# EPFL-VILAB/omnidata

Measured on AMD Instinct MI355X. Metric: images/sec (384x384) DPT-Hybrid surface-normal inference, higher is better.
Workload: dtype bf16; 1 GPU; DPT-Hybrid-384 normal, batch 32/GPU, bf16, 1xMI355X (BASELINE.json configs[1]); batch_per_gpu=32, global_batch=32, parallelism=replicas x1 (no collective in the loop), ranks_seen=1, inflight=1

## Files before the change

### include/dptx.h

```cpp
#ifndef DPTX_H_
#define DPTX_H_

#include <stddef.h>
#include <stdint.h>

#ifdef __cplusplus
extern "C" {
#endif

typedef struct dptx_engine* dptx_handle;

enum {
  DPTX_OK = 0,
  DPTX_E_INVALID = -1,
  DPTX_E_KEY = -2,
  DPTX_E_HIP = -3,
  DPTX_E_NODEVICE = -4,
  DPTX_E_ALLOC = -5
};

enum { DPTX_DTYPE_BF16 = 0, DPTX_DTYPE_FP16 = 1, DPTX_DTYPE_BF16X3 = 2,
       DPTX_DTYPE_FP16X3 = 3, DPTX_DTYPE_MIXED = 4,
       DPTX_DTYPE_FP8 = 5 };
enum { DPTX_GROUP_RESNET = 1,
// ... 225 lines not shown
int dptx_debug_arena_read(dptx_handle h, void* dst_host, size_t offset, size_t bytes);
int dptx_debug_arena_layout(dptx_handle h, char* dst, size_t capacity);
int dptx_debug_arena_checksums(dptx_handle h, void* out_dev, int32_t capacity, void* stream);
int dptx_debug_set_gemm_flags(int32_t flags);
int dptx_op_conv_fp8(const void* X8, const void* Wt8, const float* bias, const void* R, void* Y, void* Y8, int32_t B,
                     int32_t H, int32_t W, int32_t Cin, int32_t Cout, int32_t ksize, int32_t stride, int32_t pad_t,
                     int32_t pad_l, int32_t Ho, int32_t Wo, int32_t act, int32_t q_relu, float out_scale, void* stream);
int dptx_op_conv_groupnorm(int32_t dtype, const void* X, const void* Wt, void* Yraw, const float* gamma, const float* beta,
                           const void* R, void* Y, int32_t B, int32_t H, int32_t W, int32_t Cin, int32_t Cout,
                           int32_t ksize, int32_t stride, int32_t pad_t, int32_t pad_l, int32_t Ho, int32_t Wo,
                           int32_t relu, float eps, void* scratch_f32, void* stream);
int dptx_op_conv_groupnorm_fused(int32_t dtype, const void* X, const void* Wt, const float* gamma, const float* beta,
                                 const void* R, const float* r_gamma, const float* r_beta, const float* r_records, void* Y,
                                 int32_t B, int32_t H, int32_t W, int32_t Cin, int32_t Cout, int32_t relu, float eps,
                                 void* records_f32, void* tables_f32, int32_t passes, void* stream);
int dptx_op_upsample2x(int32_t dtype, const void* X, void* Y, int32_t B, int32_t H, int32_t W,
                       int32_t C, void* stream);
int dptx_op_gemm_ln(int32_t dtype, const void* A, const void* W, const float* bias, void* C, int32_t M, int32_t N, int32_t K,
                    int32_t act, const float* ln_stats, const float* ln_colsum, int32_t ln_nblk, float ln_eps, void* stream);
int dptx_op_gemm_stream(int32_t dtype, const void* A, const void* W, const float* bias, void* C, float* row_stats, int32_t M,
                        int32_t N, int32_t K, void* stream);
int dptx_op_gemm_stream32(int32_t dtype, const void* A, const void* W, const float* bias, float* X, void* C16, float* row_stats,
                          int32_t M, int32_t N, int32_t K, void* stream);
int dptx_op_head_tail(int32_t dtype, const void* H0, const void* W2, const float* b2, const float* w4,
                      const float* b4, float* y, int32_t B, int32_t Hs, int32_t Ws, int32_t C,
                      int32_t relu_out, void* stream);

typedef struct dptx_unet_engine* dptx_unet_handle;
typedef struct dptx_unet_config {
  int32_t out_channels;
// ... 40 lines not shown
```

### omnidata_amd/build.py

```python
from __future__ import annotations

import os
import subprocess
import sys

HERE = os.path.dirname(os.path.abspath(__file__))
CSRC = os.path.join(HERE, "csrc")
LIB = os.path.join(HERE, "libdptx.so")
SOURCES = ["gemm.hip", "gemm_fp16.hip", "gemm_fp16e.hip", "gemm_x3.hip", "gemm_x2.hip", "gemm_fp8.hip", "conv1x1.hip", "attention.hip", "norm.hip", "misc.hip", "stem.hip", "head.hip", "prepost.hip", "prepost_batch.hip", "fullframe.hip", "refocus.hip", "midas_loss.hip", "vnl_loss.hip", "normal_loss.hip", "eval_metrics.hip", "unet.hip", "unet_engine.hip", "engine.hip", "ops.hip"]
HEADERS = ["common.h", "kernels.h", "gemm_impl.h", "select.h", "unet.h", "resample_batch.h", os.path.join("..", "..", "include", "dptx.h")]
_NOPK = ["-Xclang", "-target-feature", "-Xclang", "-packed-fp32-ops"]
SOURCE_FLAGS = {src: list(_NOPK) for src in ("norm.hip", "misc.hip", "gemm.hip", "gemm_fp16.hip", "gemm_fp16e.hip", "gemm_x3.hip",
                                             "gemm_x2.hip", "gemm_fp8.hip", "conv1x1.hip", "refocus.hip",
                                             "midas_loss.hip", "vnl_loss.hip", "normal_loss.hip", "eval_metrics.hip",
                                             "prepost_batch.hip", "fullframe.hip", "unet.hip")}
EXPERIMENT_HEADERS = []


def source_hash(extra_flags=()) -> str:
    import hashlib
    h = hashlib.sha256()
    for name in sorted(SOURCES + HEADERS + EXPERIMENT_HEADERS):
        path = os.path.join(CSRC, name)
        h.update(os.path.basename(name).encode() + b"\0")
        with open(path, "rb") as f:
# ... 80 lines not shown
```

### omnidata_amd/csrc/conv1x1.hip

```cpp
#include "gemm_impl.h"

namespace dptx {

constexpr int C1_STG_PITCH = 144;
constexpr int C1_STG_WAVE = 16 * C1_STG_PITCH;
constexpr int C1_WAVES = 4;

template <int KT, int BN>
constexpr size_t conv1x1_smem_bytes() {
  return (size_t)KT * BN * 128 + (size_t)C1_WAVES * KT * 32 * 128 + (size_t)C1_WAVES * C1_STG_WAVE;
}

template <int DT>
__device__ __forceinline__ void c1_unpack8(const u32x4_t v, float* f) {
#pragma unroll
  for (int i = 0; i < 4; ++i) {
    f[2 * i] = T16<DT>::tof((uint16_t)(v[i] & 0xffffu));
    f[2 * i + 1] = T16<DT>::tof((uint16_t)(v[i] >> 16));
  }
}

template <int DT, int KT, int BN, int FORM>
__global__ __launch_bounds__(64 * C1_WAVES, KT <= 2 ? 2 : 1) void conv1x1_stream_kernel(const GemmParams p) {
#if defined(__HIP_DEVICE_COMPILE__)
// ... 175 lines not shown
            if (p.act == 1) {
#pragma unroll
              for (int e = 0; e < 8; ++e) f[e] = fmaxf(f[e], 0.f);
            }
#pragma unroll
            for (int e = 0; e < 4; ++e) d[e] = T16<DT>::pack2(f[2 * e], f[2 * e + 1]);
          }
          if (FORM == C1_GN || m < p.M) *(u32x4_t*)((uint16_t*)p.C + (long long)(p.c_row_off + m) * p.ldc + (n0 + s * 64 + cn * 8)) = d;
        }
      }
    }
  }
#endif
}

bool conv1x1_stream_eligible(int mode, const GemmParams& p) {
  if (mode != MODE_BF16 && mode != MODE_FP16) return false;
  if (p.ksz != 1 || p.pad_t != 0 || p.pad_l != 0 || (p.stride != 1 && p.stride != 2)) return false;
  if (p.K != p.Cin || (p.K != 64 && p.K != 128 && p.K != 256) || p.N % 64 != 0) return false;
  if (p.a_fp32 || p.c_fp32 || p.epi2 || p.a_relu || p.R1 != nullptr || p.R2 != nullptr || p.bias_per_img) return false;
  if (p.c_rpi != 0x7fffffff || p.C8 != nullptr || p.C16 != nullptr || p.out_scale != 0.f) return false;
  if (p.row_stats != nullptr || p.ln_stats != nullptr || (p.act != 0 && p.act != 1)) return false;
  if (p.ldc % 8 != 0 || p.a_pix_stride % 8 != 0 || p.a_off % 8 != 0 || p.a_img_stride % 8 != 0) return false;
  if (p.a_bytes <= 0 || p.a_bytes >= (1ll << 31) || (long long)p.N * p.ldw * 2 >= (1ll << 31) || p.M >= (1 << 23)) return false;
  return true;
}

bool conv1x1_stream_adopted(const GemmParams& p) {
  if (p.stride != 1) return false;
  if (p.K == 64) return p.N == 256 || p.N == 64;
// ... 1 lines not shown
  if (p.K == 256) return p.N == 64 || p.N == 128 || (p.N == 256 && p.a_rpi >= 48 * 48);
  return false;
}

bool conv1x1_gn_eligible(int mode, const GemmParams& p) {
  if (!conv1x1_stream_eligible(mode, p) || p.stride != 1 || p.bias != nullptr || p.act != 0) return false;
  const int cpg = p.N / 32;
  if (p.a_rpi % 32 != 0 || p.M % p.a_rpi != 0 || p.N > 1024 || (cpg & (cpg - 1)) != 0) return false;
  return p.c_row_off == 0 && p.ldc == p.N;
}

bool conv1x1_gn_adopted(const GemmParams& p) {
  if (p.K == 64) return p.N == 256;
  if (p.K == 128) return p.N == 512;
  return false;
}

template <int DT, int KT, int BN, int FORM>
static hipError_t launch_c1(const GemmParams& p, hipStream_t stream) {
  constexpr size_t smem = conv1x1_smem_bytes<KT, BN>();
  static_assert(smem <= 160 * 1024 && (KT > 2 || 2 * smem <= 160 * 1024), "two blocks per CU at K <= 128");
  const int npan = p.N / BN;
  const int rb_total = (p.M + 31) / 32;
  const int want = (rb_total + C1_WAVES - 1) / C1_WAVES;
  int cap = (KT <= 2 ? 512 : 256) / npan;
  if (cap < 8) cap = 8;
  int groups = want < cap ? want : cap;
  groups = (groups + 7) / 8 * 8;
  auto k = conv1x1_stream_kernel<DT, KT, BN, FORM>;
  set_smem_attr(k, smem);
// ... 6 lines not shown
  if (p.K == 64) {
    if constexpr (FORM != C1_GN)
      if (p.N % 256 == 0) return launch_c1<DT, 1, 256, FORM>(p, stream);
    if (p.N % 128 == 0) return launch_c1<DT, 1, 128, FORM>(p, stream);
    return launch_c1<DT, 1, 64, FORM>(p, stream);
  }
  if (p.K == 128) return p.N % 128 == 0 ? launch_c1<DT, 2, 128, FORM>(p, stream) : launch_c1<DT, 2, 64, FORM>(p, stream);
  return p.N % 128 == 0 ? launch_c1<DT, 4, 128, FORM>(p, stream) : launch_c1<DT, 4, 64, FORM>(p, stream);
}

template <int FORM>
static hipError_t launch_c1_form(int mode, const GemmParams& p, hipStream_t stream) {
  return mode == MODE_BF16 ? launch_c1_dt<DT_BF16, FORM>(p, stream) : launch_c1_dt<DT_FP16, FORM>(p, stream);
}

hipError_t launch_conv1x1_stream(int mode, const GemmParams& p0, hipStream_t stream, int form) {
  if (form == C1_PLAIN) {
    if (!conv1x1_stream_eligible(mode, p0) || p0.gn_tab != nullptr) return hipErrorInvalidValue;
    return launch_c1_form<C1_PLAIN>(mode, p0, stream);
  }
  GemmParams p = p0;
  p.trace = nullptr;
  p.a_rpi_rcp = 1.0f / (float)(p.a_rpi > 0 ? p.a_rpi : 1);
  p.wout_rcp = 1.0f / (float)(p.Wout > 0 ? p.Wout : 1);
  GemmParams q = p;
  q.R1 = nullptr; q.act = 0; q.gn_tab = nullptr; q.gn_tab_rgn = 0; q.r1_fp32 = 0;
  if (p.M <= 0 || p.ldw < p.K || p.ldw % 8 != 0 || !conv1x1_gn_eligible(mode, q) || p.r1_fp32) return hipErrorInvalidValue;
  p.gn_hw = p.a_rpi; p.gn_blocks = p.a_rpi / 32; p.gn_cpg = p.N / 32;
  if (form == C1_STATS) {
    if (p.gn_part == nullptr || p.R1 != nullptr || p.act != 0 || p.gn_tab != nullptr) return hipErrorInvalidValue;
    return launch_c1_form<C1_STATS>(mode, p, stream);
  }
  if (form != C1_GN || p.gn_tab == nullptr || p.gn_part != nullptr || p.C == nullptr || p.C == p.R1) return hipErrorInvalidValue;
  return launch_c1_form<C1_GN>(mode, p, stream);
}

}
```

### omnidata_amd/csrc/engine.hip

```cpp
#include <hip/hip_runtime.h>

#include <algorithm>
#include <cmath>
#include <cstdio>
#include <chrono>
#include <cstring>
#include <map>
#include <memory>
#include <string>
#include <unordered_map>
#include <vector>

#include "../../include/dptx.h"
#include "kernels.h"

using namespace dptx;

namespace {

constexpr int IMG = 384;
constexpr int S_TOK = 577;
constexpr int FEAT = 256;
const int STAGE_DEPTH[3] = {3, 4, 9};
const int STAGE_OUT[3] = {256, 512, 1024};
// ... 784 lines not shown
    q.gn_part = part;
    exec_macs += macs; cat_macs[0] += macs;
    chk(launch_conv1x1_stream(dt, q, st, C1_STATS), (wkey + ".stats").c_str(), 0);
    const bool r_gn = !rkey.empty();
    chk(launch_gn_finalize(part, e->f(nkey + ".weight"), e->f(nkey + ".bias"), r_gn ? rpart : nullptr,
                           r_gn ? e->f(rkey + ".weight") : nullptr, r_gn ? e->f(rkey + ".bias") : nullptr, tab, B, H * W, Cout,
                           H * W / 32, 1e-5f, st),
        (nkey + ".finalize").c_str(), 2);
    q = p;
    q.R1 = R; q.act = relu; q.gn_tab = tab; q.gn_tab_rgn = r_gn;
    exec_macs += macs; cat_macs[0] += macs;
    chk(launch_conv1x1_stream(dt, q, st, C1_GN), wkey.c_str(), 0);
    return true;
  }

  void rcu(const std::string& p, const void* x, int H, int W, void* tmp, void* out, const GemmOpt& o) {
    const int mid_lo = e->mixed() ? (int)e->layer_reads_lo(p + "conv2.weight", cur_group) : -1;
    conv(x, H, W, FEAT, p + "conv1.weight", 3, 1, 1, 1, H, W, FEAT, tmp,
         GemmOpt().bias(e->f(p + "conv1.bias")).act(1).a_relu(1).q(e->fp8_use(p + "conv2.weight") ? 1 : 0).out_lo(mid_lo));
    conv(tmp, H, W, FEAT, p + "conv2.weight", 3, 1, 1, 1, H, W, FEAT, out,
         GemmOpt().bias(e->f(p + "conv2.bias")).R1(x).R2(o.R2_).q(o.q_).out_lo(e->mixed() ? o.out_lo_ : -1));
  }

  int forward(const void* x, void* y, void* y2);
};

int Run::forward(const void* x, void* y, void* y2) {
  dptx_engine* E = e;
  E->taps.clear();
  E->event_cat.clear();
// ... 43 lines not shown
      const int stride = (b == 0) ? STAGE_STRIDE[s] : 1;
      const int Ho = H / stride, Wo = Wd / stride;
      void* out = (b == STAGE_DEPTH[s] - 1) ? (void*)A(E->S[s]) : (void*)((b & 1) ? A(E->PB) : A(E->PA));
      const bool f_in = gn_fusable(H * Wd), f_out = gn_fusable(Ho * Wo);
      if (b == 0) {
        conv(cur, H, Wd, cin, p + "downsample.conv.weight", 1, stride, 0, 0, Ho, Wo, cout, A(E->DS), GemmOpt().gn_part(f_out ? part3 : nullptr));
        if (!f_out) gn_stats(A(E->DS), part3, Ho * Wo, cout);
      }
      conv(cur, H, Wd, cin, p + "conv1.weight", 1, 1, 0, 0, H, Wd, mid, A(E->T1), GemmOpt().gn_part(f_in ? part0 : nullptr));
      if (!f_in) gn_stats(A(E->T1), part0, H * Wd, mid);
      gn_apply(A(E->T1), p + "norm1", part0, H * Wd, mid, 1);
      const int pad = (stride == 1) ? 1 : 0;
      conv(A(E->T1), H, Wd, mid, p + "conv2.weight", 3, stride, pad, pad, Ho, Wo, mid, A(E->T2), GemmOpt().gn_part(f_out ? part1 : nullptr));
      if (!f_out) gn_stats(A(E->T2), part1, Ho * Wo, mid);
      gn_apply(A(E->T2), p + "norm2", part1, Ho * Wo, mid, 1);
      const bool folded = b == 0 ? conv_gn_folded(A(E->T2), Ho, Wo, mid, p + "conv3.weight", cout, out, p + "norm3", part2, 1, A(E->DS),
                                                  p + "downsample.norm", part3)
                                 : conv_gn_folded(A(E->T2), Ho, Wo, mid, p + "conv3.weight", cout, out, p + "norm3", part2, 1, cur);
      if (!folded) {
        conv(A(E->T2), Ho, Wo, mid, p + "conv3.weight", 1, 1, 0, 0, Ho, Wo, cout, out, GemmOpt().gn_part(f_out ? part2 : nullptr));
        if (!f_out) gn_stats(out, part2, Ho * Wo, cout);
        if (b == 0)
          gn_apply(out, p + "norm3", part2, Ho * Wo, cout, 1, A(E->DS), p + "downsample.norm", part3);
        else
          gn_apply(out, p + "norm3", part2, Ho * Wo, cout, 1, cur);
      }
      cur = out;
      H = Ho;
      Wd = Wo;
      cin = cout;
    }
    const char* names[3] = {"s0", "s1", "s2"};
    tap(names[s], cur, H, Wd, cout);
// ... 921 lines not shown
```

### omnidata_amd/csrc/gemm_impl.h

```cpp
#pragma once
#include <cstdlib>
#include <type_traits>

#include "common.h"
#include "kernels.h"

namespace dptx {

constexpr int BK = 64;

__device__ __forceinline__ int row_div(int m, int d, float rcp, bool big, int& rem) {
  if (big) {
    const int q = m / d;
    rem = m - q * d;
    return q;
  }
  int q = (int)((float)m * rcp);
  int r = m - q * d;
  if (r < 0) { --q; r += d; }
  if (r >= d) { ++q; r -= d; }
  rem = r;
  return q;
}

// ... 106 lines not shown
          if (XT == 3) acc[i][j] = T16<DT>::mfma32(al[s_][i], bf[s_][j], acc[i][j]);
          acc[i][j] = T16<DT>::mfma32(af[s_][i], bl[s_][j], acc[i][j]);
          acc[i][j] = T16<DT>::mfma32(af[s_][i], bf[s_][j], acc[i][j]);
        }
      }
    };
    read(0, 0);
#pragma unroll
    for (int ks = 0; ks < BK / 16; ++ks) {
      if (ks + 1 < BK / 16) read((ks + 1) & 1, ks + 1);
      __builtin_amdgcn_sched_barrier(0);
      mma(ks & 1);
      __builtin_amdgcn_sched_barrier(0);
    }
  }
}

template <int TM, int TN>
__device__ __forceinline__ void gn_records(const GemmParams& p, int m0, int n0, int wm, int wn, int lr, int lh,
                                           f32x16_t (&acc)[TM][TN]) {
  const int cpg = p.gn_cpg;
  const int cpg_sh = __builtin_ctz(cpg);
  int gn_hw = p.gn_hw;
  asm volatile("" : "+s"(gn_hw));
#pragma unroll
  for (int i = 0; i < TM; ++i) {
    const int mb = m0 + (wm * TM + i) * 32;
    const int img = mb / gn_hw;
    const int blk = (mb - img * gn_hw) >> 5;
#pragma unroll
    for (int j = 0; j < TN; ++j) {
      float sm = 0.f, sq = 0.f;
#pragma unroll
      for (int r = 0; r < 16; ++r) { const float v = acc[i][j][r]; sm += v; sq = fmaf(v, v, sq); }
      sm += __shfl_xor(sm, 32, 64);
      sq += __shfl_xor(sq, 32, 64);
      for (int o = 1; o < cpg; o <<= 1) { sm += __shfl_xor(sm, o, 64); sq += __shfl_xor(sq, o, 64); }
      if (lh == 0 && (lr & (cpg - 1)) == 0 && mb < p.M) {
        const int g = (n0 + (wn * TN + j) * 32 + lr) >> cpg_sh;
        float2* dst = (float2*)p.gn_part + ((long long)img * p.gn_blocks + blk) * 32 + g;
        *dst = make_float2(sm, sq);
      }
    }
  }
}

template <int DT, int BM, int BN, int TM, int TN, int PL = 1, int NT = 256, int SLABS = 1, bool WP = false>
__device__ __forceinline__ void epilogue(const GemmParams& p, char* smem, int m0, int n0, int wm, int wn, int lr, int lh,
                                         int tid, f32x16_t (&acc)[TM][TN], int row_pitch = 0, bool dma_in_flight = false,
                                         int trace_row = -1, const char* lds_ln = nullptr) {
  static_assert(SLABS == 1 || SLABS == TM, "one slab, or one per MFMA row tile");
  static_assert(!WP || (SLABS == TM && TN == 2), "wave-private staging: one 32 x 64 block per wave and slab");
  constexpr int CT_PITCH = WP ? 72 : BN + 4;
  constexpr int CT_ROWS = WP ? 32 : BM / SLABS;
  constexpr int NCH = WP ? 8 : BN / 8;
  constexpr int RPP = WP ? 8 : NT / NCH;
// ... 1292 lines not shown
```

### omnidata_amd/csrc/kernels.h

```cpp
#pragma once
#include <hip/hip_runtime.h>
#include <stdint.h>

#include "common.h"

namespace dptx {

void ensure_dyn_smem(const void* kernel, size_t bytes);

struct GemmParams {
  const void* A;
  const void* W;
  void* C;
  const float* bias;
  const void* R1;
  const void* R2;
  int M, N, K;
  int ldw;
  int a_rpi, Wout, Hin, Win, Cin, a_pix_stride;
  long long a_img_stride, a_off;
  long long a_bytes;
  int ksz, stride, pad_t, pad_l;
  int c_rpi, c_img_rows, c_row_off, ldc;
  int r2_bcast;
// ... 26 lines not shown
  int debug_flags;
  float a_rpi_rcp, wout_rcp;
  const float* gn_tab;
  int gn_tab_rgn;
};

void gemm_params_dense(GemmParams& p, int M, int N, int K);
void gemm_params_conv(GemmParams& p, int B, int Hin, int Win, int Cin, int Cout, int ksz, int stride, int pad_t, int pad_l,
                      int Hout, int Wout, int a_elem_bytes);
hipError_t launch_gemm(int dtype, const GemmParams& p, hipStream_t stream);
void gemm_set_trace(long long* dev_buf);
void gemm_set_debug_flags(int flags);
int gemm_debug_flags();
bool conv1x1_stream_eligible(int mode, const GemmParams& p);
bool conv1x1_stream_adopted(const GemmParams& p);
enum { C1_PLAIN = 0, C1_STATS = 1, C1_GN = 2 };
bool conv1x1_gn_eligible(int mode, const GemmParams& p);
bool conv1x1_gn_adopted(const GemmParams& p);
hipError_t launch_conv1x1_stream(int mode, const GemmParams& p, hipStream_t stream, int form = C1_PLAIN);
void gemm_set_cu_share(float share);

hipError_t launch_attention(int mode, const void* qkv, void* out, int B, int S, int heads, Planes pl, hipStream_t stream);

hipError_t launch_layernorm(int mode, const float* x, const float* gamma, const float* beta, void* y,
                            int M, int C, float eps, Planes pl, hipStream_t stream);

struct GnParams {
  const void* X; void* Y;
  const float* gamma; const float* beta;
  float* partial;
  const void* R;
  const float* r_gamma; const float* r_beta; const float* r_partial;
  int B, HW, C, relu;
  float eps;
// ... 43 lines not shown
```

### omnidata_amd/csrc/norm.hip

```cpp
#include "common.h"
#include "kernels.h"

namespace dptx {

template <int DT, int PL, int VPL>
__global__ __launch_bounds__(256) void layernorm_kernel(const float* __restrict__ x, const float* __restrict__ gamma,
                                                        const float* __restrict__ beta, uint16_t* __restrict__ y,
                                                        int M, int C, float eps, long long plane) {
  const int lane = threadIdx.x & 63;
  const int row = blockIdx.x * 4 + (threadIdx.x >> 6);
  if (row >= M) return;
  const float* xr = x + (long long)row * C;
  float4 v[VPL];
  float s = 0.f;
#pragma unroll
  for (int j = 0; j < VPL; ++j) {
    v[j] = *(const float4*)(xr + (j * 64 + lane) * 4);
    s += (v[j].x + v[j].y) + (v[j].z + v[j].w);
  }
  const float mean = wave_sum(s) / (float)C;
  float q = 0.f;
#pragma unroll
  for (int j = 0; j < VPL; ++j) {
    const float a = v[j].x - mean, b = v[j].y - mean, c = v[j].z - mean, d = v[j].w - mean;
// ... 98 lines not shown
  if (C % 64 != 0 || C > 1024 || (256 % (C / 8)) != 0) return hipErrorInvalidValue;
  dim3 grid(gn_chunks(HW, C), B);
  DPTX_DISPATCH_MODE(mode, hipLaunchKernelGGL((gn_stats_kernel<DT, PL>), grid, dim3(256), 0, stream, (const uint16_t*)X, partial,
                                              HW, C, gn_pix(C), pl.act));
  return hipGetLastError();
}

__device__ __forceinline__ void gn_affine_to_lds(const float* __restrict__ partial, int nchunks, int b,
                                                 const float* __restrict__ gamma, const float* __restrict__ beta, int C,
                                                 int HW, float eps, float* sa, float* sd, float* smr) {
  __shared__ double sred[8][GN_G][2];
  const int tid = threadIdx.x;
  const int cpg = C >> 5;
  {
    const int g = tid & (GN_G - 1), slice = tid >> 5;
    double ss = 0.0, qq = 0.0;
    const float2* pp = (const float2*)partial + (long long)b * nchunks * GN_G + g;
    for (int c = slice; c < nchunks; c += 8) {
      const float2 v = pp[(long long)c * GN_G];
      ss += (double)v.x;
      qq += (double)v.y;
    }
    sred[slice][g][0] = ss;
    sred[slice][g][1] = qq;
  }
  __syncthreads();
  if (tid < GN_G) {
    double ss = 0.0, qq = 0.0;
#pragma unroll
    for (int sl = 0; sl < 8; ++sl) { ss += sred[sl][tid][0]; qq += sred[sl][tid][1]; }
    const double n = (double)HW * (double)cpg;
    const double mean = ss / n;
    double var = qq / n - mean * mean;
    if (var < 0.0) var = 0.0;
    smr[2 * tid] = (float)mean;
    smr[2 * tid + 1] = (float)(1.0 / sqrt(var + (double)eps));
  }
  __syncthreads();
  for (int c = tid; c < C; c += blockDim.x) {
    const int g = c / cpg;
    const float a = __fmul_rn(smr[2 * g + 1], gamma[c]);
    sa[c] = a;
    sd[c] = __builtin_fmaf(-a, smr[2 * g], beta[c]);
  }
  __syncthreads();
}

template <int DT, int PL>
__global__ __launch_bounds__(256) void gn_apply_kernel(const GnParams p, int pix, int nrec, long long plane) {
  __shared__ float sa[1024], sd[1024], ra[1024], rd[1024], smr[64];
  const int b = blockIdx.y;
  gn_affine_to_lds(p.partial, nrec, b, p.gamma, p.beta, p.C, p.HW, p.eps, sa, sd, smr);
  const bool r_gn = (p.R != nullptr) && (p.r_gamma != nullptr);
  if (r_gn) gn_affine_to_lds(p.r_partial, nrec, b, p.r_gamma, p.r_beta, p.C, p.HW, p.eps, ra, rd, smr);
  const int cvec = p.C >> 3;
  const int pbeg = blockIdx.x * pix;
  const int pend = min(pbeg + pix, p.HW);
  const long long img = (long long)b * p.HW * p.C;
// ... 117 lines not shown
```

### omnidata_amd/csrc/ops.hip

```cpp
#include <hip/hip_runtime.h>

#include "../../include/dptx.h"
#include "kernels.h"

using namespace dptx;

extern "C" {

static int rc(hipError_t r) { return r == hipSuccess ? DPTX_OK : DPTX_E_HIP; }

static Planes g_op_planes{0, 0};
int dptx_op_set_planes(int64_t act_plane_elems, int64_t w_plane_elems) {
  g_op_planes.act = act_plane_elems;
  g_op_planes.w = w_plane_elems;
  return DPTX_OK;
}

int dptx_op_gemm(int32_t dtype, const void* A, const void* W, const float* bias, const void* R, void* C, int32_t M, int32_t N,
                 int32_t K, int32_t act, int32_t a_fp32, int32_t c_fp32, int32_t r_fp32, void* stream) {
  GemmParams p;
  gemm_params_dense(p, M, N, K);
  p.A = A; p.W = W; p.C = C; p.bias = bias; p.R1 = R; p.act = act; p.a_fp32 = a_fp32; p.c_fp32 = c_fp32; p.r1_fp32 = r_fp32;
  p.planes = g_op_planes;
  return rc(launch_gemm(dtype, p, (hipStream_t)stream));
// ... 141 lines not shown
    if (launch_conv1x1_stream(dtype, q, st, C1_STATS) != hipSuccess) return DPTX_E_HIP;
  }
  if (passes & 2) {
    if (launch_gn_finalize((const float*)records_f32, gamma, beta, r_records, r_gamma, r_beta, (float*)tables_f32, B, H * W, Cout,
                           H * W / 32, eps, st) != hipSuccess)
      return DPTX_E_HIP;
  }
  if (passes & 4) {
    GemmParams q = p;
    q.R1 = R; q.act = relu ? 1 : 0; q.gn_tab = (const float*)tables_f32; q.gn_tab_rgn = r_gamma != nullptr;
    if (launch_conv1x1_stream(dtype, q, st, C1_GN) != hipSuccess) return DPTX_E_HIP;
  }
  return DPTX_OK;
}

int dptx_op_upsample2x(int32_t dtype, const void* X, void* Y, int32_t B, int32_t H, int32_t W, int32_t C, void* stream) {
  return rc(launch_upsample2x(dtype, X, Y, B, H, W, C, g_op_planes, (hipStream_t)stream));
}

}
```

### omnidata_amd/engine.py

```python
from __future__ import annotations

import ctypes as C
import os
from typing import Dict, Optional, Tuple

import numpy as np
import torch

_HERE = os.path.dirname(os.path.abspath(__file__))
LIB_PATH = os.environ.get("DPTX_LIB") or os.path.join(_HERE, "libdptx.so")

DTYPES = {"bf16": 0, "fp16": 1, "bf16x3": 2, "fp16x3": 3, "mixed": 4, "fp8": 5}
TWO_PLANE_DTYPES = frozenset(("bf16x3", "fp16x3", "mixed", "fp8"))
GROUPS = {"resnet": 1, "embed": 2, "vit": 4, "reassemble": 8, "rn": 16, "fusion": 32, "head": 64, "all": 127}
FLAGS = {"no_ln_fold": 1, "group_policy": 2, "fp32_stream": 4, "no_range_check": 8, "fp8_all": 16, "fp8_vit": 32}


def groups_mask(names) -> int:
    if isinstance(names, int):
        return names
    if isinstance(names, str):
        names = [n for n in names.replace(",", "+").split("+") if n]
    mask = 0
    for n in names:
# ... 95 lines not shown
    ("dptx_op_stem_conv", C.c_int, [_i32, _vp, _vp, _vp, _i32, _i32, _i32, _vp]),
    ("dptx_op_attention", C.c_int, [_i32, _vp, _vp, _i32, _i32, _i32, _vp]),
    ("dptx_op_layernorm", C.c_int, [_i32, _vp, _vp, _vp, _vp, _i32, _i32, C.c_float, _vp]),
    ("dptx_op_groupnorm", C.c_int, [_i32, _vp, _vp, _vp, _vp, _vp, _i32, _i32, _i32, _i32, C.c_float, _vp, _vp]),
    ("dptx_op_gn_relu_maxpool", C.c_int, [_i32, _vp, _vp, _vp, _vp, _i32, _i32, _i32, _i32, C.c_float, _vp, _vp]),
    ("dptx_op_cls_rows", C.c_int, [_i32, _vp, _vp, _vp, _i32, _i32, _i32, _vp, _vp, _vp, C.c_float, _vp]),
    ("dptx_debug_set_trace", C.c_int, [_vp]),
    ("dptx_debug_set_gemm_flags", C.c_int, [C.c_int32]),
    ("dptx_debug_arena_fill", C.c_int, [_vp, _i32]),
    ("dptx_debug_arena_read", C.c_int, [_vp, _vp, _sz, _sz]),
    ("dptx_debug_arena_layout", C.c_int, [_vp, C.c_char_p, _sz]),
    ("dptx_debug_arena_checksums", C.c_int, [_vp, _vp, _i32, _vp]),
    ("dptx_op_conv_fp8", C.c_int, [_vp, _vp, _vp, _vp, _vp, _vp] + [_i32] * 13 + [C.c_float, _vp]),
    ("dptx_op_conv_groupnorm", C.c_int, [_i32, _vp, _vp, _vp, _vp, _vp, _vp, _vp] + [_i32] * 12 + [C.c_float, _vp, _vp]),
    ("dptx_op_conv_groupnorm_fused", C.c_int, [_i32] + [_vp] * 9 + [_i32] * 6 + [C.c_float, _vp, _vp, _i32, _vp]),
    ("dptx_op_upsample2x", C.c_int, [_i32, _vp, _vp, _i32, _i32, _i32, _i32, _vp]),
    ("dptx_op_gemm_ln", C.c_int, [_i32, _vp, _vp, _vp, _vp, _i32, _i32, _i32, _i32, _vp, _vp, _i32, C.c_float, _vp]),
    ("dptx_op_gemm_stream", C.c_int, [_i32, _vp, _vp, _vp, _vp, _vp, _i32, _i32, _i32, _vp]),
    ("dptx_op_gemm_stream32", C.c_int, [_i32, _vp, _vp, _vp, _vp, _vp, _vp, _i32, _i32, _i32, _vp]),
    ("dptx_op_head_tail", C.c_int, [_i32, _vp, _vp, _vp, _vp, _vp, _vp, _i32, _i32, _i32, _i32, _i32, _vp]),
    ("dptx_unet_default_config", None, [_vp]),
    ("dptx_unet_create", C.c_int, [C.POINTER(_vp), _vp]),
    ("dptx_unet_destroy", None, [_vp]),
    ("dptx_unet_last_error", C.c_char_p, [_vp]),
    ("dptx_unet_load_tensor", C.c_int, [_vp, C.c_char_p, _vp, _i64p, _i32]),
    ("dptx_unet_finalize_weights", C.c_int, [_vp]),
    ("dptx_unet_packed_bytes", _sz, [_vp]),
    ("dptx_unet_packed_entry", C.c_int, [_vp, C.c_char_p, _i64p, _i64p]),
    ("dptx_unet_export_packed_host", C.c_int, [_vp, _vp, _sz]),
    ("dptx_unet_device_bytes", _sz, [_vp]),
# ... 368 lines not shown
```

Measured before the change: 2868 images/s.

## Fuse 1x1 conv with whole-image GroupNorm in a single per-image kernel

```diff
diff --git a/include/dptx.h b/include/dptx.h
--- a/include/dptx.h
+++ b/include/dptx.h
@@ -263,6 +263,9 @@
                                  const void* R, const float* r_gamma, const float* r_beta, const float* r_records, void* Y,
                                  int32_t B, int32_t H, int32_t W, int32_t Cin, int32_t Cout, int32_t relu, float eps,
                                  void* records_f32, void* tables_f32, int32_t passes, void* stream);
+int dptx_op_conv_groupnorm_image(int32_t dtype, const void* X, const void* Wt, const float* gamma, const float* beta,
+                                 const void* R, const float* r_gamma, const float* r_beta, const float* r_records, void* Y,
+                                 int32_t B, int32_t H, int32_t W, int32_t Cin, int32_t Cout, int32_t relu, float eps, void* stream);
 int dptx_op_upsample2x(int32_t dtype, const void* X, void* Y, int32_t B, int32_t H, int32_t W,
                        int32_t C, void* stream);
 int dptx_op_gemm_ln(int32_t dtype, const void* A, const void* W, const float* bias, void* C, int32_t M, int32_t N, int32_t K,
diff --git a/omnidata_amd/build.py b/omnidata_amd/build.py
--- a/omnidata_amd/build.py
+++ b/omnidata_amd/build.py
@@ -8,7 +8,7 @@
 CSRC = os.path.join(HERE, "csrc")
 LIB = os.path.join(HERE, "libdptx.so")
 SOURCES = ["gemm.hip", "gemm_fp16.hip", "gemm_fp16e.hip", "gemm_x3.hip", "gemm_x2.hip", "gemm_fp8.hip", "conv1x1.hip", "attention.hip", "norm.hip", "misc.hip", "stem.hip", "head.hip", "prepost.hip", "prepost_batch.hip", "fullframe.hip", "refocus.hip", "midas_loss.hip", "vnl_loss.hip", "normal_loss.hip", "eval_metrics.hip", "unet.hip", "unet_engine.hip", "engine.hip", "ops.hip"]
-HEADERS = ["common.h", "kernels.h", "gemm_impl.h", "select.h", "unet.h", "resample_batch.h", os.path.join("..", "..", "include", "dptx.h")]
+HEADERS = ["common.h", "kernels.h", "gemm_impl.h", "gn_affine.h", "select.h", "unet.h", "resample_batch.h", os.path.join("..", "..", "include", "dptx.h")]
 _NOPK = ["-Xclang", "-target-feature", "-Xclang", "-packed-fp32-ops"]
 SOURCE_FLAGS = {src: list(_NOPK) for src in ("norm.hip", "misc.hip", "gemm.hip", "gemm_fp16.hip", "gemm_fp16e.hip", "gemm_x3.hip",
                                              "gemm_x2.hip", "gemm_fp8.hip", "conv1x1.hip", "refocus.hip",
diff --git a/omnidata_amd/csrc/conv1x1.hip b/omnidata_amd/csrc/conv1x1.hip
--- a/omnidata_amd/csrc/conv1x1.hip
+++ b/omnidata_amd/csrc/conv1x1.hip
@@ -1,4 +1,5 @@
 #include "gemm_impl.h"
+#include "gn_affine.h"
 
 namespace dptx {
 
@@ -213,6 +214,268 @@
 #endif
 }
 
+constexpr int C1_IMG_RB = 5;
+constexpr int C1_IMG_REC = C1_WAVES * C1_IMG_RB;
+constexpr int C1_IMG_MAX_ROWS = C1_IMG_REC * 32;
+
+struct C1ImgArgs {
+  const float *gamma, *beta;
+  const float *r_gamma, *r_beta, *r_part;
+  float eps;
+};
+
+template <int KT>
+constexpr size_t conv1x1_img_smem_bytes() {
+  return (size_t)KT * 64 * 128 + (size_t)C1_WAVES * KT * 32 * 128 + (size_t)C1_WAVES * C1_STG_WAVE;
+}
+
+template <int KT>
+__device__ __forceinline__ void c1_issue_a(const GemmParams& p, const __amdgpu_buffer_rsrc_t rsrcA, char* sa, int lane, int rblk) {
+  const int kc = lane & 7, r0 = lane >> 3;
+#pragma unroll
+  for (int i = 0; i < 4; ++i) {
+    const int row = r0 + 8 * i;
+    const int m = rblk * 32 + row;
+    const bool ok = m < p.M;
+    const int mm = ok ? m : 0;
+    int rem, ox;
+    const int img = row_div(mm, p.a_rpi, p.a_rpi_rcp, false, rem);
+    const int oy = row_div(rem, p.Wout, p.wout_rcp, false, ox);
+    const int iy = oy * p.stride - p.pad_t, ix = ox * p.stride - p.pad_l;
+    const bool valid = ok && ((unsigned)iy < (unsigned)p.Hin) && ((unsigned)ix < (unsigned)p.Win);
+    const long long e = (long long)img * p.a_img_stride + p.a_off + ((long long)iy * p.Win + ix) * p.a_pix_stride +
+                        (kc ^ ((row >> 1) & 7)) * 8;
+    const unsigned base = (unsigned)(e * 2);
+#pragma unroll
+    for (int kt = 0; kt < KT; ++kt) {
+      const unsigned vo = valid ? base + kt * 128 : OOB;
+      __builtin_amdgcn_raw_ptr_buffer_load_lds(rsrcA, (__attribute__((address_space(3))) void*)(sa + kt * 4096 + i * 1024), 16, vo,
+                                               0, 0, 0);
+    }
+  }
+}
+
+template <int DT, int KT>
+__global__ __launch_bounds__(64 * C1_WAVES, 1) void conv1x1_image_kernel(const GemmParams p, const C1ImgArgs g) {
+#if defined(__HIP_DEVICE_COMPILE__)
+  constexpr int BN = 64;
+  constexpr int KS = KT * 4;
+  constexpr int W_BYTES = KT * BN * 128;
+  constexpr int A_WAVE = KT * 32 * 128;
+  constexpr int RB = C1_IMG_RB;
+  extern __shared__ __attribute__((aligned(16))) char smem[];
+  __shared__ float2 s_rec[C1_IMG_REC][32];
+  __shared__ double s_red[2][8][32][2];
+  __shared__ float s_mr[2][64];
+  __shared__ float s_aff[4][BN];
+
+  const int tid = threadIdx.x;
+  const int lane = tid & 63;
+  const int wave = __builtin_amdgcn_readfirstlane(tid >> 6);
+  const int lr = lane & 31, lh = lane >> 5;
+
+  const int npan = p.N / BN;
+  const int x = (int)blockIdx.x & 7, l = (int)blockIdx.x >> 3;
+  const int img = (l / npan) * 8 + x;
+  const int n0 = (l % npan) * BN;
+  const int nrb = p.gn_blocks;
+  if (img * p.gn_hw >= p.M) return;
+  const int rbase = img * nrb;
+
+  const int cpg = p.gn_cpg, cpg_sh = __builtin_ctz(cpg);
+  const int gpp = BN >> cpg_sh;
+  const bool has_r = p.R1 != nullptr;
+  const bool r_gn = has_r && g.r_part != nullptr;
+
+  const int w_bytes = (int)((long long)p.N * p.ldw * 2);
+  const __amdgpu_buffer_rsrc_t rsrcA = __builtin_amdgcn_make_buffer_rsrc(const_cast<void*>(p.A), 0, (int)p.a_bytes, 0x00020000);
+  const __amdgpu_buffer_rsrc_t rsrcW = __builtin_amdgcn_make_buffer_rsrc(const_cast<void*>(p.W), 0, w_bytes, 0x00020000);
+  char* const sw = smem;
+  char* const sa = smem + W_BYTES + wave * A_WAVE;
+  char* const stg = smem + W_BYTES + C1_WAVES * A_WAVE + wave * C1_STG_WAVE;
+
+  if (wave < nrb) c1_issue_a<KT>(p, rsrcA, sa, lane, rbase + wave);
+  {
+    const int kc = lane & 7, r0 = lane >> 3;
+    for (int idx = wave; idx < KT * (BN / 8); idx += C1_WAVES) {
+      const int kt = idx / (BN / 8), rg = idx - kt * (BN / 8);
+      const int row = rg * 8 + r0;
+      const unsigned vo = (unsigned)(((long long)(n0 + row) * p.ldw + kt * 64 + (kc ^ ((row >> 1) & 7)) * 8) * 2);
+      __builtin_amdgcn_raw_ptr_buffer_load_lds(rsrcW, (__attribute__((address_space(3))) void*)(sw + kt * (BN * 128) + rg * 1024), 16,
+                                               vo, 0, 0, 0);
+    }
+  }
+  const int sg = tid & 31, slice = tid >> 5;
+  const int at = tid >> 6, ac = tid & 63;
+  float gam = 0.f, bet = 0.f;
+  if (at == 0 || (at == 1 && r_gn)) {
+    gam = (at ? g.r_gamma : g.gamma)[n0 + ac];
+    bet = (at ? g.r_beta : g.beta)[n0 + ac];
+  }
+  if (r_gn && sg < gpp) {
+    double ss, qq;
+    gn_slice_sums((const float2*)g.r_part + (long long)rbase * 32 + (n0 >> cpg_sh) + sg, 32, nrb, slice, ss, qq);
+    s_red[1][slice][sg][0] = ss;
+    s_red[1][slice][sg][1] = qq;
+  }
+  asm volatile("s_waitcnt vmcnt(0)" ::: "memory");
+  __syncthreads();
+
+  const int swz = (lr >> 1) & 7;
+  const unsigned sel = (lr & 1) ? 0x03020706u : 0x05040100u;
+  const int cn = lane & 7, rr = lane >> 3;
+
+  uint32_t pk[RB][2][8];
+  u32x4_t rq[RB][4];
+  float2 rs[RB * 2];
+#pragma unroll
+  for (int n = 0; n < RB * 2; ++n) rs[n] = make_float2(0.f, 0.f);
+#pragma unroll
+  for (int i = 0; i < RB; ++i) {
+    const int rb = wave + C1_WAVES * i;
+    if (rb < nrb) {
+      const int m0 = (rbase + rb) * 32;
+      u32x4_t af[KS];
+#pragma unroll
+      for (int ks = 0; ks < KS; ++ks)
+        af[ks] = *(const u32x4_t*)(sa + (ks >> 2) * 4096 + lr * 128 + (((2 * (ks & 3) + lh) ^ swz) << 4));
+      asm volatile("s_waitcnt lgkmcnt(0)" ::: "memory");
+      const bool prefetch = rb + C1_WAVES < nrb;
+      if (prefetch) c1_issue_a<KT>(p, rsrcA, sa, lane, rbase + rb + C1_WAVES);
+      asm volatile("" ::: "memory");
+      if (has_r) {
+#pragma unroll
+        for (int q = 0; q < 4; ++q) {
+          const int m = m0 + 16 * (q >> 1) + rr + 8 * (q & 1);
+          rq[i][q] = *(const u32x4_t*)((const uint16_t*)p.R1 + (long long)m * p.ldc + (n0 + cn * 8));
+        }
+      }
+      asm volatile("" ::: "memory");
+
+      f32x16_t acc[2];
+#pragma unroll
+      for (int j = 0; j < 2; ++j)
+#pragma unroll
+        for (int r = 0; r < 16; ++r) acc[j][r] = 0.f;
+      u32x4_t bf[2][4][2];
+      auto read_w = [&](int kt) {
+#pragma unroll
+        for (int q = 0; q < 4; ++q)
+#pragma unroll
+          for (int j = 0; j < 2; ++j)
+            bf[kt & 1][q][j] = *(const u32x4_t*)(sw + kt * (BN * 128) + (j * 32 + lr) * 128 + (((2 * q + lh) ^ swz) << 4));
+      };
+      read_w(0);
+#pragma unroll
+      for (int kt = 0; kt < KT; ++kt) {
+        if (kt + 1 < KT) read_w(kt + 1);
+        __builtin_amdgcn_sched_barrier(0);
+#pragma unroll
+        for (int q = 0; q < 4; ++q)
+#pragma unroll
+          for (int j = 0; j < 2; ++j) acc[j] = T16<DT>::mfma32(af[kt * 4 + q], bf[kt & 1][q][j], acc[j]);
+      }
+      __builtin_amdgcn_sched_barrier(0);
+#pragma unroll
+      for (int j = 0; j < 2; ++j) {
+        rs[2 * i + j] = gn_record_rows(acc[j]);
+#pragma unroll
+        for (int t = 0; t < 8; ++t) pk[i][j][t] = T16<DT>::pack2(acc[j][2 * t], acc[j][2 * t + 1]);
+      }
+      if (prefetch) {
+        if (has_r) asm volatile("s_waitcnt vmcnt(4)" ::: "memory");
+        else asm volatile("s_waitcnt vmcnt(0)" ::: "memory");
+      }
+    }
+  }
+  gn_record_lanes<RB * 2>(rs, cpg);
+#pragma unroll
+  for (int i = 0; i < RB; ++i) {
+    const int rb = wave + C1_WAVES * i;
+#pragma unroll
+    for (int j = 0; j < 2; ++j)
+      if (rb < nrb && lh == 0 && (lr & (cpg - 1)) == 0) s_rec[rb][(j * 32 + lr) >> cpg_sh] = rs[2 * i + j];
+  }
+  __syncthreads();
+
+  if (sg < gpp) {
+    double ss, qq;
+    gn_slice_sums(&s_rec[0][sg], 32, nrb, slice, ss, qq);
+    s_red[0][slice][sg][0] = ss;
+    s_red[0][slice][sg][1] = qq;
+  }
+  __syncthreads();
+  if (tid < 64 && sg < gpp && (slice == 0 || r_gn))
+    gn_mean_rstd(&s_red[slice][0][sg][0], 64, p.gn_hw, cpg, g.eps, s_mr[slice][2 * sg], s_mr[slice][2 * sg + 1]);
+  __syncthreads();
+  if (at == 0 || (at == 1 && r_gn)) {
+    const int gg = ac >> cpg_sh;
+    gn_channel_affine(s_mr[at][2 * gg], s_mr[at][2 * gg + 1], gam, bet, s_aff[2 * at][ac], s_aff[2 * at + 1][ac]);
+  }
+  __syncthreads();
+
+  float ga[8], gd[8], gra[8], grd[8];
+#pragma unroll
+  for (int e = 0; e < 8; ++e) {
+    ga[e] = s_aff[0][cn * 8 + e];
+    gd[e] = s_aff[1][cn * 8 + e];
+    gra[e] = r_gn ? s_aff[2][cn * 8 + e] : 0.f;
+    grd[e] = r_gn ? s_aff[3][cn * 8 + e] : 0.f;
+  }
+#pragma unroll
+  for (int i = 0; i < RB; ++i) {
+    const int rb = wave + C1_WAVES * i;
+    if (rb < nrb) {
+      const int m0 = (rbase + rb) * 32;
+#pragma unroll
+      for (int h = 0; h < 2; ++h) {
+        asm volatile("" ::: "memory");
+        __builtin_amdgcn_wave_barrier();
+#pragma unroll
+        for (int j = 0; j < 2; ++j)
+#pragma unroll
+          for (int t = 0; t < 4; ++t) {
+            const uint32_t own = pk[i][j][4 * h + t];
+            const uint32_t nb = (uint32_t)__builtin_amdgcn_update_dpp(0, (int)own, 0xB1, 0xf, 0xf, false);
+            const uint32_t o = __builtin_amdgcn_perm(nb, own, sel);
+            const int rl = ((2 * t) & 3) + (lr & 1) + 8 * (t >> 1) + 4 * lh;
+            *(uint32_t*)(stg + rl * C1_STG_PITCH + (j * 32 + (lr & ~1)) * 2) = o;
+          }
+        asm volatile("" ::: "memory");
+        __builtin_amdgcn_wave_barrier();
+#pragma unroll
+        for (int pp = 0; pp < 2; ++pp) {
+          const int rl = rr + 8 * pp;
+          u32x4_t d = *(const u32x4_t*)(stg + rl * C1_STG_PITCH + cn * 16);
+          const int m = m0 + 16 * h + rl;
+          float f[8];
+          c1_unpack8<DT>(d, f);
+#pragma unroll
+          for (int e = 0; e < 8; ++e) f[e] = __builtin_fmaf(f[e], ga[e], gd[e]);
+          if (has_r) {
+            float r[8];
+            c1_unpack8<DT>(rq[i][2 * h + pp], r);
+            if (r_gn) {
+#pragma unroll
+              for (int e = 0; e < 8; ++e) r[e] = __builtin_fmaf(r[e], gra[e], grd[e]);
+            }
+#pragma unroll
+            for (int e = 0; e < 8; ++e) f[e] = __fadd_rn(f[e], r[e]);
+          }
+          if (p.act == 1) {
+#pragma unroll
+            for (int e = 0; e < 8; ++e) f[e] = fmaxf(f[e], 0.f);
+          }
+#pragma unroll
+          for (int e = 0; e < 4; ++e) d[e] = T16<DT>::pack2(f[2 * e], f[2 * e + 1]);
+          *(u32x4_t*)((uint16_t*)p.C + (long long)m * p.ldc + (n0 + cn * 8)) = d;
+        }
+      }
+    }
+  }
+#endif
+}
+
 bool conv1x1_stream_eligible(int mode, const GemmParams& p) {
   if (mode != MODE_BF16 && mode != MODE_FP16) return false;
   if (p.ksz != 1 || p.pad_t != 0 || p.pad_l != 0 || (p.stride != 1 && p.stride != 2)) return false;
@@ -244,6 +507,33 @@
   if (p.K == 64) return p.N == 256;
   if (p.K == 128) return p.N == 512;
   return false;
+}
+
+bool conv1x1_gn_image_eligible(int mode, const GemmParams& p) {
+  return conv1x1_gn_eligible(mode, p) && p.a_rpi <= C1_IMG_MAX_ROWS;
+}
+
+bool conv1x1_gn_image_adopted(const GemmParams& p) {
+  return p.K == 256 && p.N == 1024 && p.a_rpi <= C1_IMG_MAX_ROWS;
+}
+
+template <int DT, int KT>
+static hipError_t launch_c1_img(const GemmParams& p, const C1ImgArgs& g, hipStream_t stream) {
+  constexpr size_t smem = conv1x1_img_smem_bytes<KT>();
+  static_assert(smem + 16 * 1024 <= 160 * 1024, "dynamic + static LDS of conv1x1_image_kernel");
+  const int npan = p.N / 64;
+  const int nimg = p.M / p.a_rpi;
+  auto k = conv1x1_image_kernel<DT, KT>;
+  set_smem_attr(k, smem);
+  hipLaunchKernelGGL(k, dim3((nimg + 7) / 8 * 8 * npan), dim3(64 * C1_WAVES), smem, stream, p, g);
+  return hipGetLastError();
+}
+
+template <int DT>
+static hipError_t launch_c1_img_dt(const GemmParams& p, const C1ImgArgs& g, hipStream_t stream) {
+  if (p.K == 64) return launch_c1_img<DT, 1>(p, g, stream);
+  if (p.K == 128) return launch_c1_img<DT, 2>(p, g, stream);
+  return launch_c1_img<DT, 4>(p, g, stream);
 }
 
 template <int DT, int KT, int BN, int FORM>
@@ -280,7 +570,7 @@
   return mode == MODE_BF16 ? launch_c1_dt<DT_BF16, FORM>(p, stream) : launch_c1_dt<DT_FP16, FORM>(p, stream);
 }
 
-hipError_t launch_conv1x1_stream(int mode, const GemmParams& p0, hipStream_t stream, int form) {
+hipError_t launch_conv1x1_stream(int mode, const GemmParams& p0, hipStream_t stream, int form, const GnParams* gn) {
   if (form == C1_PLAIN) {
     if (!conv1x1_stream_eligible(mode, p0) || p0.gn_tab != nullptr) return hipErrorInvalidValue;
     return launch_c1_form<C1_PLAIN>(mode, p0, stream);
@@ -293,6 +583,13 @@
   q.R1 = nullptr; q.act = 0; q.gn_tab = nullptr; q.gn_tab_rgn = 0; q.r1_fp32 = 0;
   if (p.M <= 0 || p.ldw < p.K || p.ldw % 8 != 0 || !conv1x1_gn_eligible(mode, q) || p.r1_fp32) return hipErrorInvalidValue;
   p.gn_hw = p.a_rpi; p.gn_blocks = p.a_rpi / 32; p.gn_cpg = p.N / 32;
+  if (form == C1_IMG) {
+    if (gn == nullptr || gn->gamma == nullptr || gn->beta == nullptr || !conv1x1_gn_image_eligible(mode, q)) return hipErrorInvalidValue;
+    if (p.gn_part != nullptr || p.gn_tab != nullptr || p.C == nullptr || p.C == p.R1) return hipErrorInvalidValue;
+    if (gn->r_partial != nullptr && (p.R1 == nullptr || gn->r_gamma == nullptr || gn->r_beta == nullptr)) return hipErrorInvalidValue;
+    const C1ImgArgs g{gn->gamma, gn->beta, gn->r_gamma, gn->r_beta, gn->r_partial, gn->eps};
+    return mode == MODE_BF16 ? launch_c1_img_dt<DT_BF16>(p, g, stream) : launch_c1_img_dt<DT_FP16>(p, g, stream);
+  }
   if (form == C1_STATS) {
     if (p.gn_part == nullptr || p.R1 != nullptr || p.act != 0 || p.gn_tab != nullptr) return hipErrorInvalidValue;
     return launch_c1_form<C1_STATS>(mode, p, stream);
diff --git a/omnidata_amd/csrc/engine.hip b/omnidata_amd/csrc/engine.hip
--- a/omnidata_amd/csrc/engine.hip
+++ b/omnidata_amd/csrc/engine.hip
@@ -822,6 +822,25 @@
     return true;
   }
 
+  bool conv_gn_image(const void* in, int H, int W, int Cin, const std::string& wkey, int Cout, void* out, const std::string& nkey,
+                     int relu, const void* R, const std::string& rkey = "", const float* rpart = nullptr) {
+    const int flags = gemm_debug_flags();
+    if ((flags & (8 | 32 | 64)) || !gn_fusable(H * W) || out == R || (e->fp8_use(wkey) && !e->calibrating)) return false;
+    GemmParams p;
+    gemm_params_conv(p, B, H, W, Cin, Cout, 1, 1, 0, 0, H, W, 2);
+    p.A = in; p.W = e->w(wkey); p.C = out; p.planes = e->pl;
+    if (!conv1x1_gn_image_eligible(dt, p) || !((flags & 128) || conv1x1_gn_image_adopted(p))) return false;
+    const bool r_gn = !rkey.empty();
+    GnParams g{};
+    g.gamma = e->f(nkey + ".weight"); g.beta = e->f(nkey + ".bias"); g.eps = 1e-5f;
+    if (r_gn) { g.r_gamma = e->f(rkey + ".weight"); g.r_beta = e->f(rkey + ".bias"); g.r_partial = rpart; }
+    p.R1 = R; p.act = relu;
+    const double macs = (double)p.M / B * p.N * p.K;
+    exec_macs += macs; cat_macs[0] += macs;
+    chk(launch_conv1x1_stream(dt, p, st, C1_IMG, &g), wkey.c_str(), 0);
+    return true;
+  }
+
   void rcu(const std::string& p, const void* x, int H, int W, void* tmp, void* out, const GemmOpt& o) {
     const int mid_lo = e->mixed() ? (int)e->layer_reads_lo(p + "conv2.weight", cur_group) : -1;
     conv(x, H, W, FEAT, p + "conv1.weight", 3, 1, 1, 1, H, W, FEAT, tmp,
@@ -895,9 +914,11 @@
       conv(A(E->T1), H, Wd, mid, p + "conv2.weight", 3, stride, pad, pad, Ho, Wo, mid, A(E->T2), GemmOpt().gn_part(f_out ? part1 : nullptr));
       if (!f_out) gn_stats(A(E->T2), part1, Ho * Wo, mid);
       gn_apply(A(E->T2), p + "norm2", part1, Ho * Wo, mid, 1);
-      const bool folded = b == 0 ? conv_gn_folded(A(E->T2), Ho, Wo, mid, p + "conv3.weight", cout, out, p + "norm3", part2, 1, A(E->DS),
-                                                  p + "downsample.norm", part3)
-                                 : conv_gn_folded(A(E->T2), Ho, Wo, mid, p + "conv3.weight", cout, out, p + "norm3", part2, 1, cur);
+      const void* R = b == 0 ? (const void*)A(E->DS) : cur;
+      const std::string rkey = b == 0 ? p + "downsample.norm" : std::string();
+      const float* rpart = b == 0 ? part3 : nullptr;
+      const bool folded = conv_gn_image(A(E->T2), Ho, Wo, mid, p + "conv3.weight", cout, out, p + "norm3", 1, R, rkey, rpart) ||
+                          conv_gn_folded(A(E->T2), Ho, Wo, mid, p + "conv3.weight", cout, out, p + "norm3", part2, 1, R, rkey, rpart);
       if (!folded) {
         conv(A(E->T2), Ho, Wo, mid, p + "conv3.weight", 1, 1, 0, 0, Ho, Wo, cout, out, GemmOpt().gn_part(f_out ? part2 : nullptr));
         if (!f_out) gn_stats(out, part2, Ho * Wo, cout);
diff --git a/omnidata_amd/csrc/gemm_impl.h b/omnidata_amd/csrc/gemm_impl.h
--- a/omnidata_amd/csrc/gemm_impl.h
+++ b/omnidata_amd/csrc/gemm_impl.h
@@ -144,6 +144,30 @@
       __builtin_amdgcn_sched_barrier(0);
     }
   }
+}
+
+__device__ __forceinline__ float2 gn_record_rows(const f32x16_t& a) {
+  float sm = 0.f, sq = 0.f;
+#pragma unroll
+  for (int r = 0; r < 16; ++r) { const float v = a[r]; sm += v; sq = fmaf(v, v, sq); }
+  return make_float2(sm, sq);
+}
+template <int NREC>
+__device__ __forceinline__ void gn_record_lanes(float2 (&s)[NREC], int cpg) {
+#pragma unroll
+  for (int n = 0; n < NREC; ++n) {
+    s[n].x += __shfl_xor(s[n].x, 32, 64);
+    s[n].y += __shfl_xor(s[n].y, 32, 64);
+  }
+  for (int o = 1; o < cpg; o <<= 1) {
+#pragma unroll
+    for (int n = 0; n < NREC; ++n) { s[n].x += __shfl_xor(s[n].x, o, 64); s[n].y += __shfl_xor(s[n].y, o, 64); }
+  }
+}
+__device__ __forceinline__ float2 gn_record_sums(const f32x16_t& a, int cpg) {
+  float2 s[1] = {gn_record_rows(a)};
+  gn_record_lanes<1>(s, cpg);
+  return s[0];
 }
 
 template <int TM, int TN>
@@ -160,16 +184,11 @@
     const int blk = (mb - img * gn_hw) >> 5;
 #pragma unroll
     for (int j = 0; j < TN; ++j) {
-      float sm = 0.f, sq = 0.f;
-#pragma unroll
-      for (int r = 0; r < 16; ++r) { const float v = acc[i][j][r]; sm += v; sq = fmaf(v, v, sq); }
-      sm += __shfl_xor(sm, 32, 64);
-      sq += __shfl_xor(sq, 32, 64);
-      for (int o = 1; o < cpg; o <<= 1) { sm += __shfl_xor(sm, o, 64); sq += __shfl_xor(sq, o, 64); }
+      const float2 rec = gn_record_sums(acc[i][j], cpg);
       if (lh == 0 && (lr & (cpg - 1)) == 0 && mb < p.M) {
         const int g = (n0 + (wn * TN + j) * 32 + lr) >> cpg_sh;
         float2* dst = (float2*)p.gn_part + ((long long)img * p.gn_blocks + blk) * 32 + g;
-        *dst = make_float2(sm, sq);
+        *dst = rec;
       }
     }
   }
diff --git a/omnidata_amd/csrc/gn_affine.h b/omnidata_amd/csrc/gn_affine.h
--- /dev/null
+++ b/omnidata_amd/csrc/gn_affine.h
@@ -0,0 +1,33 @@
+#pragma once
+#include "common.h"
+
+namespace dptx {
+
+__device__ __forceinline__ void gn_slice_sums(const float2* rec, int stride, int nrec, int slice, double& ss, double& qq) {
+  ss = 0.0;
+  qq = 0.0;
+  for (int c = slice; c < nrec; c += 8) {
+    const float2 v = rec[(long long)c * stride];
+    ss += (double)v.x;
+    qq += (double)v.y;
+  }
+}
+
+__device__ __forceinline__ void gn_mean_rstd(const double* sred, int stride, int HW, int cpg, float eps, float& mean, float& rstd) {
+  double ss = 0.0, qq = 0.0;
+#pragma unroll
+  for (int sl = 0; sl < 8; ++sl) { ss += sred[sl * stride]; qq += sred[sl * stride + 1]; }
+  const double n = (double)HW * (double)cpg;
+  const double m = ss / n;
+  double var = qq / n - m * m;
+  if (var < 0.0) var = 0.0;
+  mean = (float)m;
+  rstd = (float)(1.0 / sqrt(var + (double)eps));
+}
+
+__device__ __forceinline__ void gn_channel_affine(float mean, float rstd, float gamma, float beta, float& a, float& d) {
+  a = __fmul_rn(rstd, gamma);
+  d = __builtin_fmaf(-a, mean, beta);
+}
+
+}
diff --git a/omnidata_amd/csrc/kernels.h b/omnidata_amd/csrc/kernels.h
--- a/omnidata_amd/csrc/kernels.h
+++ b/omnidata_amd/csrc/kernels.h
@@ -64,10 +64,13 @@
 int gemm_debug_flags();
 bool conv1x1_stream_eligible(int mode, const GemmParams& p);
 bool conv1x1_stream_adopted(const GemmParams& p);
-enum { C1_PLAIN = 0, C1_STATS = 1, C1_GN = 2 };
+enum { C1_PLAIN = 0, C1_STATS = 1, C1_GN = 2, C1_IMG = 3 };
+struct GnParams;
 bool conv1x1_gn_eligible(int mode, const GemmParams& p);
 bool conv1x1_gn_adopted(const GemmParams& p);
-hipError_t launch_conv1x1_stream(int mode, const GemmParams& p, hipStream_t stream, int form = C1_PLAIN);
+bool conv1x1_gn_image_eligible(int mode, const GemmParams& p);
+bool conv1x1_gn_image_adopted(const GemmParams& p);
+hipError_t launch_conv1x1_stream(int mode, const GemmParams& p, hipStream_t stream, int form = C1_PLAIN, const GnParams* gn = nullptr);
 void gemm_set_cu_share(float share);
 
 hipError_t launch_attention(int mode, const void* qkv, void* out, int B, int S, int heads, Planes pl, hipStream_t stream);
diff --git a/omnidata_amd/csrc/norm.hip b/omnidata_amd/csrc/norm.hip
--- a/omnidata_amd/csrc/norm.hip
+++ b/omnidata_amd/csrc/norm.hip
@@ -1,4 +1,5 @@
 #include "common.h"
+#include "gn_affine.h"
 #include "kernels.h"
 
 namespace dptx {
@@ -136,34 +137,17 @@
   const int cpg = C >> 5;
   {
     const int g = tid & (GN_G - 1), slice = tid >> 5;
-    double ss = 0.0, qq = 0.0;
-    const float2* pp = (const float2*)partial + (long long)b * nchunks * GN_G + g;
-    for (int c = slice; c < nchunks; c += 8) {
-      const float2 v = pp[(long long)c * GN_G];
-      ss += (double)v.x;
-      qq += (double)v.y;
-    }
+    double ss, qq;
+    gn_slice_sums((const float2*)partial + (long long)b * nchunks * GN_G + g, GN_G, nchunks, slice, ss, qq);
     sred[slice][g][0] = ss;
     sred[slice][g][1] = qq;
   }
   __syncthreads();
-  if (tid < GN_G) {
-    double ss = 0.0, qq = 0.0;
-#pragma unroll
-    for (int sl = 0; sl < 8; ++sl) { ss += sred[sl][tid][0]; qq += sred[sl][tid][1]; }
-    const double n = (double)HW * (double)cpg;
-    const double mean = ss / n;
-    double var = qq / n - mean * mean;
-    if (var < 0.0) var = 0.0;
-    smr[2 * tid] = (float)mean;
-    smr[2 * tid + 1] = (float)(1.0 / sqrt(var + (double)eps));
-  }
+  if (tid < GN_G) gn_mean_rstd(&sred[0][tid][0], GN_G * 2, HW, cpg, eps, smr[2 * tid], smr[2 * tid + 1]);
   __syncthreads();
   for (int c = tid; c < C; c += blockDim.x) {
     const int g = c / cpg;
-    const float a = __fmul_rn(smr[2 * g + 1], gamma[c]);
-    sa[c] = a;
-    sd[c] = __builtin_fmaf(-a, smr[2 * g], beta[c]);
+    gn_channel_affine(smr[2 * g], smr[2 * g + 1], gamma[c], beta[c], sa[c], sd[c]);
   }
   __syncthreads();
 }
diff --git a/omnidata_amd/csrc/ops.hip b/omnidata_amd/csrc/ops.hip
--- a/omnidata_amd/csrc/ops.hip
+++ b/omnidata_amd/csrc/ops.hip
@@ -179,6 +179,23 @@
   return DPTX_OK;
 }
 
+int dptx_op_conv_groupnorm_image(int32_t dtype, const void* X, const void* Wt, const float* gamma, const float* beta, const void* R,
+                                 const float* r_gamma, const float* r_beta, const float* r_records, void* Y, int32_t B, int32_t H,
+                                 int32_t W, int32_t Cin, int32_t Cout, int32_t relu, float eps, void* stream) {
+  if (X == nullptr || Wt == nullptr || gamma == nullptr || beta == nullptr || Y == nullptr || Y == R || B <= 0 || H <= 0 || W <= 0)
+    return DPTX_E_INVALID;
+  if ((r_gamma != nullptr) != (r_beta != nullptr) || (r_gamma != nullptr) != (r_records != nullptr)) return DPTX_E_INVALID;
+  if (r_gamma != nullptr && R == nullptr) return DPTX_E_INVALID;
+  GemmParams p;
+  gemm_params_conv(p, B, H, W, Cin, Cout, 1, 1, 0, 0, H, W, 2);
+  p.A = X; p.W = Wt; p.C = Y; p.planes = g_op_planes;
+  if (!conv1x1_gn_image_eligible(dtype, p)) return DPTX_E_INVALID;
+  GnParams g{};
+  g.gamma = gamma; g.beta = beta; g.r_gamma = r_gamma; g.r_beta = r_beta; g.r_partial = r_records; g.eps = eps;
+  p.R1 = R; p.act = relu ? 1 : 0;
+  return rc(launch_conv1x1_stream(dtype, p, (hipStream_t)stream, C1_IMG, &g));
+}
+
 int dptx_op_upsample2x(int32_t dtype, const void* X, void* Y, int32_t B, int32_t H, int32_t W, int32_t C, void* stream) {
   return rc(launch_upsample2x(dtype, X, Y, B, H, W, C, g_op_planes, (hipStream_t)stream));
 }
diff --git a/omnidata_amd/engine.py b/omnidata_amd/engine.py
--- a/omnidata_amd/engine.py
+++ b/omnidata_amd/engine.py
@@ -133,6 +133,7 @@
     ("dptx_op_conv_fp8", C.c_int, [_vp, _vp, _vp, _vp, _vp, _vp] + [_i32] * 13 + [C.c_float, _vp]),
     ("dptx_op_conv_groupnorm", C.c_int, [_i32, _vp, _vp, _vp, _vp, _vp, _vp, _vp] + [_i32] * 12 + [C.c_float, _vp, _vp]),
     ("dptx_op_conv_groupnorm_fused", C.c_int, [_i32] + [_vp] * 9 + [_i32] * 6 + [C.c_float, _vp, _vp, _i32, _vp]),
+    ("dptx_op_conv_groupnorm_image", C.c_int, [_i32] + [_vp] * 9 + [_i32] * 6 + [C.c_float, _vp]),
     ("dptx_op_upsample2x", C.c_int, [_i32, _vp, _vp, _i32, _i32, _i32, _i32, _vp]),
     ("dptx_op_gemm_ln", C.c_int, [_i32, _vp, _vp, _vp, _vp, _i32, _i32, _i32, _i32, _vp, _vp, _i32, C.c_float, _vp]),
     ("dptx_op_gemm_stream", C.c_int, [_i32, _vp, _vp, _vp, _vp, _vp, _i32, _i32, _i32, _vp]),
```

Result: no change. 2895 images/s, median of 6 (+0.9%).
